# MartinMikkelsen/TensorTrainNumerics.jl

Hardware: AMD Instinct MI355X
Metric: TT cores/sec for QTT Laplacian apply+round, d=30 rank-64 (higher is better)
Workload: dtype f64

## Files before the change

### tensortrainnumerics.jl_amd/csrc/ttn_dense_kernels.h

```cpp
#pragma once
#include "ttn_wg_prims.h"
#include "ttn_wg_gemm.h"
#include "ttn_wg_lq.h"
#include "ttn_wg_jacobi.h"
#include "ttn_wg_chol.h"

struct CompressArgs {
    TTDev tt;
    long long max_bond;
    double truncerr;
    int sweeps;
    int k_single;
    int k_first, k_last;
    double* scratch;
    long long scratch_stride;
    int pmax, qmax;
    double* sv_out;
    int sv_steps;
    int* status;
    int* sweep_stats;
    int fast;
    int fused;
    TTODev op;
    TTDev x;
// ... 260 lines not shown
        const int i = e % r, j = e / r;
        const double si = S.sigs[i], sj = S.sigs[j];
        const double ref = (i == j) ? si * s0 : 0.0;
        worst = fmax(worst, fabs(D[i + (long long)ldd * j] - ref) / (s0 * sqrt(si * sj)));
    }
    return wg_max(worst, S.red);
}

__device__ void wg_materialize_core(const CompressArgs& P, int b, int k) {
    const TTDev& T = P.tt;
    const int n = T.dims[k];
    const long long* xr = P.x.rks + (long long)b * (P.x.d + 1);
    const int rl = uni32((int)xr[k]), rr = uni32((int)xr[k + 1]);
    const int Rl = uni32((int)P.op.rks[k]), Rr = uni32((int)P.op.rks[k + 1]);
    const double* xc = P.x.data + (long long)b * P.x.stride + P.x.off[k];
    const double* ac = P.op.data + P.op.off[k];
    double* yc = T.data + (long long)b * T.stride + T.off[k];
    const long long Dl = (long long)Rl * rl, tot = (long long)n * Dl * Rr * rr;
    for (long long e = threadIdx.x; e < tot; e += TTN_WG) {
        const int s = (int)(e % n);
        const long long t1 = e / n;
        const int ga = (int)(t1 % Dl), be = (int)(t1 / Dl);
        const int a1 = ga % Rl, nu1 = ga / Rl, a2 = be % Rr, nu2 = be / Rr;
        double v = 0.0;
        for (int j = 0; j < n; ++j)
            v = fma(ac[s + n * (j + n * (a1 + (long long)Rl * a2))], xc[j + n * (nu1 + (long long)rl * nu2)], v);
        yc[e] = v;
    }
    __syncthreads();
}

#define FM_BK 8
__device__ __noinline__ bool wg_fused_merge_mfma(double* ck, const double* xc, const double* ac, double* M, int p, int q, int n1, int Dl,
                                                 int rhl, int rhr, int Rl, int Rr, double* lds, double* amax_lds, double* red) {
    ck = unip(ck); xc = unip(xc); ac = unip(ac); M = unip(M); lds = unip(lds); amax_lds = unip(amax_lds); red = unip(red);
    p = uni32(p); q = uni32(q); n1 = uni32(n1); Dl = uni32(Dl); rhl = uni32(rhl); rhr = uni32(rhr); Rl = uni32(Rl); Rr = uni32(Rr);
    constexpr int n2 = 2;
    const int tid = threadIdx.x, lane = tid & 63, wave = tid >> 6;
    const int li = lane & 15, lk = lane >> 4;
    const int RT = p >> 4;
    const int WR = RT < 8 ? RT : 8;
    const int WC = TTN_NWAVES / WR;
    const int CP = 32 * WC;
    const int ncol = n2 * rhr, nin = Rl * n2, nout = n2 * Rr;
    constexpr int LDA = GEMM_LD;
    const int LDB = (CP <= 32) ? 49 : (CP <= 64) ? 81 : GEMM_LD;
    const int stage = Rl * FM_BK * LDA + FM_BK * LDB;
    if (Rl < 1 || Rl > 3 || Rr > 4 || (p & 15) || (rhl % FM_BK) || (ncol % CP) || (RT % WR) || WR * WC != TTN_NWAVES || CP > 128 ||
        Rl * FM_BK * 16 * WR > 6 * TTN_WG || FM_BK * CP > 2 * TTN_WG || 2 * stage + 64 > GEMM_LDS_DOUBLES)
        return false;
    lds_f64* opl = (lds_f64*)lds + 2 * stage;
    __syncthreads();
    for (int e = tid; e < nin * nout; e += TTN_WG) {
        const int i = e % nin, o = e / nin;
        opl[e] = ac[(o % n2) + n2 * ((i % n2) + n2 * ((i / n2) + (long long)Rl * (o / n2)))];
    }
    const long long ldk = (long long)n1 * Dl;
    const int wr = wave % WR, wc = wave / WR;
    const int nchunk = rhl / FM_BK;
    gmem_f64* Cg = (gmem_f64*)ck;
    gmem_f64* Xg = (gmem_f64*)xc;
    gmem_wf64* Mg = (gmem_wf64*)M;
    double cmax = 0.0;
    const int arows = 16 * WR;
    const int na_el = Rl * FM_BK * arows, nb_el = FM_BK * CP;
    constexpr int NUA = 6, NUB = 2;
    for (int rb = 0; rb < RT; rb += WR) {
        for (int c0 = 0; c0 < ncol; c0 += CP) {
            mfma_acc_t acc[3][2];
#pragma unroll
            for (int a1 = 0; a1 < 3; ++a1) { acc[a1][0] = (mfma_acc_t){0.0, 0.0, 0.0, 0.0}; acc[a1][1] = (mfma_acc_t){0.0, 0.0, 0.0, 0.0}; }
            int aoff[NUA], alds[NUA], boff[NUB], blds[NUB];
            bool aok[NUA], bok[NUB];
#pragma unroll
            for (int u = 0; u < NUA; ++u) {
                const int e = tid + TTN_WG * u;
                aok[u] = e < na_el;
                const int r = e % arows, rest = e / arows, kk = rest % FM_BK, a1 = rest / FM_BK;
                const int row = 16 * rb + r;
                aoff[u] = aok[u] ? (row % Dl) * n1 + row / Dl + (int)(ldk * (a1 + (long long)Rl * kk)) : 0;
                alds[u] = (a1 * FM_BK + kk) * LDA + r;
            }
#pragma unroll
            for (int u = 0; u < NUB; ++u) {
                const int e = tid + TTN_WG * u;
                bok[u] = e < nb_el;
                const int c = e % CP, kk = e / CP, col = c0 + c;
                boff[u] = bok[u] ? (col & 1) + n2 * (kk + rhl * (col >> 1)) : 0;
                blds[u] = kk * LDB + c;
            }
            const int astep = (int)(ldk * Rl * FM_BK), bstep = n2 * FM_BK;
            double av[NUA], bv[NUB];
#define FM_LOAD(CH)                                                                                                     \
            { _Pragma("unroll") for (int u = 0; u < NUA; ++u) av[u] = Cg[aoff[u] + (CH) * astep];                       \
              _Pragma("unroll") for (int u = 0; u < NUB; ++u) bv[u] = Xg[boff[u] + (CH) * bstep]; }
#define FM_STORE(STG)                                                                                                   \
            { lds_f64* As_ = (lds_f64*)lds + (STG) * stage; lds_f64* Bs_ = As_ + Rl * FM_BK * LDA;                      \
              _Pragma("unroll") for (int u = 0; u < NUA; ++u) if (aok[u]) As_[alds[u]] = av[u];                         \
              _Pragma("unroll") for (int u = 0; u < NUB; ++u) if (bok[u]) Bs_[blds[u]] = bv[u]; }
            __syncthreads();
            FM_LOAD(0)
            FM_STORE(0)
            if (nchunk > 1) FM_LOAD(1)
            __syncthreads();
            for (int ch = 0; ch < nchunk; ++ch) {
                const lds_f64* As = (lds_f64*)lds + (ch & 1) * stage;
                const lds_f64* Bs = As + Rl * FM_BK * LDA;
#pragma unroll
                for (int t = 0; t < FM_BK / 4; ++t) {
                    const int kr = 4 * t + lk;
                    const double b0 = Bs[kr * LDB + wc * 32 + li], b1 = Bs[kr * LDB + wc * 32 + 16 + li];
#pragma unroll
                    for (int a1 = 0; a1 < 3; ++a1) {
                        if (a1 < Rl) {
                            const double a = As[(a1 * FM_BK + kr) * LDA + wr * 16 + li];
                            acc[a1][0] = __builtin_amdgcn_mfma_f64_16x16x4f64(a, b0, acc[a1][0], 0, 0, 0);
                            acc[a1][1] = __builtin_amdgcn_mfma_f64_16x16x4f64(a, b1, acc[a1][1], 0, 0, 0);
                        }
                    }
                    if (t == 0 && ch + 1 < nchunk) FM_STORE((ch + 1) & 1)
                }
                if (ch + 2 < nchunk) FM_LOAD(ch + 2)
                __syncthreads();
            }
#undef FM_LOAD
#undef FM_STORE
            const int jl = li & 1;
#pragma unroll
            for (int ct = 0; ct < 2; ++ct) {
                const int nu = (c0 + wc * 32 + ct * 16 + li) >> 1;
#pragma unroll
                for (int reg = 0; reg < 4; ++reg) {
                    const int row = 16 * (rb + wr) + lk + 4 * reg;
                    gmem_wf64* mrow = Mg + ((long long)row * q + (long long)nout * nu);
                    for (int o = 0; o < nout; ++o) {
                        double v = 0.0;
#pragma unroll
                        for (int a1 = 0; a1 < 3; ++a1)
                            if (a1 < Rl) v = fma(acc[a1][ct][reg], opl[o * nin + jl + n2 * a1], v);
                        v += dpp_mov_f64<0xB1>(v);
                        if ((o & 1) == jl) mrow[o] = v;
                        cmax = fmax(cmax, fabs(v));
                    }
                }
            }
        }
    }
    cmax = wg_max(cmax, red);
    if (tid == 0) *amax_lds = cmax;
    __syncthreads();
    return true;
}

__device__ __noinline__ bool wg_fused_merge_direct(double* ck, const double* xc, const double* ac, double* M, int p, int q, int n1, int Dl,
                                                   int rhl, int rhr, int Rl, int Rr, double* lds, double* amax_lds, double* red) {
    ck = unip(ck); xc = unip(xc); ac = unip(ac); M = unip(M); lds = unip(lds); amax_lds = unip(amax_lds); red = unip(red);
    p = uni32(p); q = uni32(q); n1 = uni32(n1); Dl = uni32(Dl); rhl = uni32(rhl); rhr = uni32(rhr); Rl = uni32(Rl); Rr = uni32(Rr);
    constexpr int n2 = 2;
    const int tid = threadIdx.x, lane = tid & 63, wave = tid >> 6;
    const int li = lane & 15, lk = lane >> 4;
    const int RT = p >> 4;
    const int WR = RT < 8 ? RT : 8;
    const int WC = TTN_NWAVES / WR;
    const int CP = 32 * WC;
    const int ncol = n2 * rhr, nin = Rl * n2, nout = n2 * Rr;
    const int LDB = ncol + 1;
    if (Rl < 1 || Rl > 3 || Rr > 4 || (p & 15) || (rhl & 15) || (ncol % CP) || (RT % WR) || WR * WC != TTN_NWAVES ||
        (long long)rhl * LDB + 64 > GEMM_LDS_DOUBLES)
        return false;
    lds_f64* Bs = (lds_f64*)lds;
    lds_f64* opl = Bs + rhl * LDB;
    gmem_f64* Cg = (gmem_f64*)ck;
    gmem_f64* Xg = (gmem_f64*)xc;
    gmem_wf64* Mg = (gmem_wf64*)M;
    __syncthreads();
    for (int e = tid; e < nin * nout; e += TTN_WG) {
        const int i = e % nin, o = e / nin;
        opl[e] = ac[(o % n2) + n2 * ((i % n2) + n2 * ((i / n2) + (long long)Rl * (o / n2)))];
    }
    {
        const int nx = rhl * ncol, kspan = n2 * rhl;
        for (int e0 = tid; e0 < nx; e0 += 8 * TTN_WG) {
            double v[8];
#pragma unroll
            for (int u = 0; u < 8; ++u) { const int e = e0 + u * TTN_WG; v[u] = Xg[e < nx ? e : e0]; }
#pragma unroll
            for (int u = 0; u < 8; ++u) {
                const int e = e0 + u * TTN_WG;
                if (e < nx) { const int nu = e / kspan, w_ = e - nu * kspan, j = w_ & 1, kk = w_ >> 1; Bs[kk * LDB + j + n2 * nu] = v[u]; }
            }
        }
    }
    __syncthreads();
    const long long ldk = (long long)n1 * Dl;
    const int wr = wave % WR, wc = wave / WR;
    const int ksteps = rhl >> 2, ngrp = ksteps >> 2;
    const int kstride = (int)(ldk * Rl);
    double cmax = 0.0;
    const int jl = li & 1;
    for (int rb = 0; rb < RT; rb += WR) {
        const int arow = 16 * (rb + wr) + li;
        const int abase = (arow % Dl) * n1 + arow / Dl + lk * kstride;
        for (int c0 = 0; c0 < ncol; c0 += CP) {
            mfma_acc_t acc[3][2];
#pragma unroll
            for (int a1 = 0; a1 < 3; ++a1) { acc[a1][0] = (mfma_acc_t){0.0, 0.0, 0.0, 0.0}; acc[a1][1] = (mfma_acc_t){0.0, 0.0, 0.0, 0.0}; }
            double cur[4][3], nxt[4][3];
#define FMD_LOAD(DST, G)                                                                                                \
            _Pragma("unroll") for (int t = 0; t < 4; ++t)                                                                \
                _Pragma("unroll") for (int a1 = 0; a1 < 3; ++a1)                                                         \
                    DST[t][a1] = (a1 < Rl) ? Cg[abase + (4 * (4 * (G) + t)) * kstride + a1 * (int)ldk] : 0.0;
            FMD_LOAD(cur, 0)
            const lds_f64* bcol = Bs + lk * LDB + c0 + wc * 32 + li;
            for (int g = 0; g < ngrp; ++g) {
                if (g + 1 < ngrp) { FMD_LOAD(nxt, g + 1) }
#pragma unroll
                for (int t = 0; t < 4; ++t) {
                    const int kr = 4 * (4 * g + t);
                    const double b0 = bcol[kr * LDB], b1 = bcol[kr * LDB + 16];
#pragma unroll
                    for (int a1 = 0; a1 < 3; ++a1) {
                        if (a1 < Rl) {
                            acc[a1][0] = __builtin_amdgcn_mfma_f64_16x16x4f64(cur[t][a1], b0, acc[a1][0], 0, 0, 0);
                            acc[a1][1] = __builtin_amdgcn_mfma_f64_16x16x4f64(cur[t][a1], b1, acc[a1][1], 0, 0, 0);
                        }
                    }
                }
#pragma unroll
                for (int t = 0; t < 4; ++t)
#pragma unroll
                    for (int a1 = 0; a1 < 3; ++a1) cur[t][a1] = nxt[t][a1];
            }
#undef FMD_LOAD
            const int half = nout >> 1;
            const bool vec_ok = (half == 3) && ((((unsigned long long)Mg) & 15ull) == 0) && ((q & 1) == 0);
            if (vec_ok && Rl == 3) {
                double w[3][3][2];
#pragma unroll
                for (int oo = 0; oo < 3; ++oo)
#pragma unroll
                    for (int a1 = 0; a1 < 3; ++a1) {
                        const int o = 3 * jl + oo;
                        w[oo][a1][0] = opl[o * nin + jl + n2 * a1];
                        w[oo][a1][1] = opl[o * nin + (1 - jl) + n2 * a1];
                    }
                typedef double dbl2 __attribute__((ext_vector_type(2)));
                typedef __attribute__((address_space(1))) dbl2 gmem_wd2;
#pragma unroll
                for (int ct = 0; ct < 2; ++ct) {
                    const int nu = (c0 + wc * 32 + ct * 16 + li) >> 1;
#pragma unroll
                    for (int reg = 0; reg < 4; ++reg) {
                        const int row = 16 * (rb + wr) + lk + 4 * reg;
                        gmem_wf64* mrow = Mg + ((long long)row * q + (long long)nout * nu);
                        const double t0 = acc[0][ct][reg], t1 = acc[1][ct][reg], t2 = acc[2][ct][reg];
                        const double u0 = dpp_mov_f64<0xB1>(t0), u1 = dpp_mov_f64<0xB1>(t1), u2 = dpp_mov_f64<0xB1>(t2);
                        double v[3];
#pragma unroll
                        for (int oo = 0; oo < 3; ++oo) {
                            double x_ = t0 * w[oo][0][0];
                            x_ = fma(u0, w[oo][0][1], x_);
                            x_ = fma(t1, w[oo][1][0], x_); x_ = fma(u1, w[oo][1][1], x_);
                            x_ = fma(t2, w[oo][2][0], x_); x_ = fma(u2, w[oo][2][1], x_);
                            v[oo] = x_;
                            cmax = fmax(cmax, fabs(x_));
                        }
                        *(gmem_wd2*)(mrow + (jl ? 4 : 0)) = jl ? (dbl2){v[1], v[2]} : (dbl2){v[0], v[1]};
                        mrow[jl ? 3 : 2] = jl ? v[0] : v[2];
                    }
                }
            } else {
#pragma unroll
            for (int ct = 0; ct < 2; ++ct) {
                const int nu = (c0 + wc * 32 + ct * 16 + li) >> 1;
#pragma unroll
                for (int reg = 0; reg < 4; ++reg) {
                    const int row = 16 * (rb + wr) + lk + 4 * reg;
                    gmem_wf64* mrow = Mg + ((long long)row * q + (long long)nout * nu);
                    for (int o = 0; o < nout; ++o) {
                        double v = 0.0;
#pragma unroll
                        for (int a1 = 0; a1 < 3; ++a1)
                            if (a1 < Rl) v = fma(acc[a1][ct][reg], opl[o * nin + jl + n2 * a1], v);
                        v += dpp_mov_f64<0xB1>(v);
                        if ((o >= half) == (jl == 1)) mrow[o] = v;
                        cmax = fmax(cmax, fabs(v));
                    }
                }
            }
            }
        }
    }
    cmax = wg_max(cmax, red);
    if (tid == 0) *amax_lds = cmax;
    __syncthreads();
    return true;
}


#define FUSE_MAX_TERMS 16
__device__ bool wg_fused_merge(const CompressArgs& P, int b, int k, int p, int q, const View& Am, double* M, double* Tbuf,
                               long long tbuf_doubles, double* lds, double* amax_lds, double* red) {
    const TTDev& T = P.tt;
    const int n1 = T.dims[k], n2 = T.dims[k + 1];
    const long long* rks = T.rks + (long long)b * (T.d + 1);
    const int Dl = uni32((int)rks[k]);
    const long long* xr = P.x.rks + (long long)b * (P.x.d + 1);
    const int rhl = uni32((int)xr[k + 1]), rhr = uni32((int)xr[k + 2]);
    const int Rl = uni32((int)P.op.rks[k + 1]), Rr = uni32((int)P.op.rks[k + 2]);
    const int ncol = n2 * rhr;
    if (Rl * n2 > FUSE_MAX_TERMS || n2 * Rr > FUSE_MAX_TERMS || (long long)Rl * p * ncol > tbuf_doubles) return false;
    if ((long long)Rl * rhl != rks[k + 1] || (long long)n2 * Rr * rhr != q || p != n1 * Dl) return false;
    double* ck = T.data + (long long)b * T.stride + T.off[k];
    double* xc = P.x.data + (long long)b * P.x.stride + P.x.off[k + 1];
    const double* ac = P.op.data + P.op.off[k + 1];
    TTN_SETPRIO_GEMM();
    struct PrioRestore { __device__ ~PrioRestore() { TTN_SETPRIO_BASE(); } } prio_restore_;
    if (n2 == 2 && wg_fused_merge_direct(ck, xc, ac, M, p, q, n1, Dl, rhl, rhr, Rl, Rr, lds, amax_lds, red)) return true;
    if (n2 == 2 && wg_fused_merge_mfma(ck, xc, ac, M, p, q, n1, Dl, rhl, rhr, Rl, Rr, lds, amax_lds, red)) return true;
    const long long ldk = (long long)n1 * Dl;
    for (int a1 = 0; a1 < Rl; ++a1) {
        const View Av = mkview(ck + a1 * ldk, Am.r, plain((long long)Rl * ldk));
        const View Bv = mkview(xc, plain(n2), Idx{n2, 1, (long long)n2 * rhl});
        const View Cv = mkview(Tbuf + (long long)a1 * p * ncol, plain(ncol), plain(1));
        wg_gemm(p, ncol, rhl, Av, Bv, Cv, 1.0, 0.0, lds);
    }
    double mx = 0.0;
    const int nin = Rl * n2, nout = n2 * Rr;
    lds_f64* opl = (lds_f64*)lds;
    for (int e = threadIdx.x; e < nin * nout; e += TTN_WG) {
        const int i = e % nin, o = e / nin;
        opl[e] = ac[(o % n2) + n2 * ((i % n2) + n2 * ((i / n2) + (long long)Rl * (o / n2)))];
    }
    __syncthreads();
    const long long tstride = (long long)p * ncol;
    for (int e = threadIdx.x; e < p * rhr; e += TTN_WG) {
        const int nu = e % rhr, row = e / rhr;
        const double* tp = Tbuf + (long long)row * ncol + n2 * nu;
        double t[FUSE_MAX_TERMS];
#pragma unroll
        for (int i = 0; i < FUSE_MAX_TERMS; ++i) t[i] = (i < nin) ? tp[(i / n2) * tstride + (i % n2)] : 0.0;
        double* mrow = M + (long long)row * q + (long long)nout * nu;
        for (int o = 0; o < nout; ++o) {
            const lds_f64* w = opl + o * nin;
            double v = 0.0;
#pragma unroll
            for (int i = 0; i < FUSE_MAX_TERMS; ++i)
                if (i < nin) v = fma(t[i], w[i], v);
            mrow[o] = v;
            mx = fmax(mx, fabs(v));
        }
    }
    mx = wg_max(mx, red);
    if (threadIdx.x == 0) *amax_lds = mx;
    __syncthreads();
    return true;
}

#define SMALL_STEP_PMAX 8
#define SMALL_STEP_QMAX 256
struct SmallStepArgs {
    double truncerr;
    long long max_bond;
    int rank_rule, pmax;
    double* sv_row;
    int* status_b;
    double *red, *scal, *sigs;
    int *perm, *iflag;
};
__device__ __noinline__ int wg_bond_small(SmallStepArgs Q, double* ck, double* ck1, int n1, int n2, int Dl, int rm, int Dr, long long* rank_out, double* lds) {
    rm = uni32(rm); n1 = uni32(n1); n2 = uni32(n2); Dl = uni32(Dl); Dr = uni32(Dr);
    ck = unip(ck); ck1 = unip(ck1); rank_out = unip(rank_out); lds = unip(lds);
    const int mr = n1 * Dl, mc = n2 * Dr;
    const View Am = mkview(ck, Idx{Dl, (long long)n1, 1}, plain((long long)n1 * Dl));
    const View Bm = mkview(ck1, plain(n2), Idx{n2, 1, (long long)n2 * rm});
    const int wide = (mr <= mc) ? 1 : 0;
    const int p = wide ? mr : mc, q = wide ? mc : mr;
    const View Ap = wide ? Am : tview(Bm);
    const View Bp = wide ? Bm : tview(Am);
    Q.truncerr = unif64(Q.truncerr); Q.max_bond = uni64(Q.max_bond);
    Q.rank_rule = uni32(Q.rank_rule); Q.pmax = uni32(Q.pmax); Q.sv_row = unip(Q.sv_row); Q.status_b = unip(Q.status_b);
    Q.red = unip(Q.red); Q.scal = unip(Q.scal); Q.sigs = unip(Q.sigs); Q.perm = unip(Q.perm); Q.iflag = unip(Q.iflag);
    const int tid = threadIdx.x, lane = tid & 63, wave = tid >> 6;
    const int LDQ = q + 1;
    lds_f64* Ms = (lds_f64*)lds;
    lds_f64* Es = Ms + SMALL_STEP_PMAX * (SMALL_STEP_QMAX + 1);
    lds_f64* nr = Es + SMALL_STEP_PMAX * 17;
    lds_i32* flg = (lds_i32*)(nr + 16);
    gmem_f64* Ag = (gmem_f64*)Ap.p;
    gmem_f64* Bg = (gmem_f64*)Bp.p;
    __syncthreads();
    double mx = 0.0;
    for (int e = tid; e < p * q; e += TTN_WG) {
        const int i = e / q, j = e - i * q;
        const long long ao = ix(Ap.r, i), bo = ix(Bp.c, j);
        double acc = 0.0;
        for (int kk = 0; kk < rm; ++kk) acc = fma(Ag[ao + ix(Ap.c, kk)], Bg[bo + ix(Bp.r, kk)], acc);
        Ms[i * LDQ + j] = acc;
        mx = fmax(mx, fabs(acc));
    }
    for (int e = tid; e < p * 17; e += TTN_WG) Es[e] = ((e / 17) == (e % 17)) ? 1.0 : 0.0;
    mx = unif64(wg_max(mx, Q.red));
    const double s0 = (mx > 0.0) ? mx : 1.0, inv_s0 = 1.0 / s0;
    for (int e = tid; e < p * q; e += TTN_WG) { const int i = e / q, j = e - i * q; Ms[i * LDQ + j] *= inv_s0; }
    __syncthreads();
    double amax = 0.0;
    for (int i = wave; i < p; i += TTN_NWAVES) {
        double a = 0.0;
        for (int j = lane; j < q; j += 64) { const double v = Ms[i * LDQ + j]; a = fma(v, v, a); }
        a = wave_sum(a);
        if (lane == 0) nr[i] = a;
        amax = fmax(amax, a);
    }
    amax = unif64(wg_max(amax, Q.red));
    const double aneg = (double)q * DBL_EPSILON * DBL_EPSILON * amax;
    const double tol = sqrt((double)q) * DBL_EPSILON, tol2 = tol * tol;
    if (tid == 0) Q.scal[0] = aneg;
    const int pe = p + (p & 1), half = pe >> 1;
    int sweeps = 0, conv = (p < 2);
    for (; !conv && sweeps < JACOBI_MAX_SWEEPS; ++sweeps) {
        if (tid == 0) *flg = 0;
        __syncthreads();
        int rotated = 0;
        for (int round = 0; round < pe - 1; ++round) {
            for (int kk = wave; kk < half; kk += TTN_NWAVES) {
                int i, j;
                if (kk == 0) { i = round; j = pe - 1; }
                else { i = (round + kk) % (pe - 1); j = (round + pe - 1 - kk) % (pe - 1); }
                if (i > j) { const int t = i; i = j; j = t; }
                if (j >= p) continue;
                lds_f64* xi = Ms + i * LDQ;
                lds_f64* xj = Ms + j * LDQ;
                double u[4], v[4];
                double a = 0.0, b_ = 0.0, g = 0.0;
#pragma unroll
                for (int t4 = 0; t4 < 4; ++t4) {
                    const int c = lane + 64 * t4;
                    u[t4] = (c < q) ? xi[c] : 0.0; v[t4] = (c < q) ? xj[c] : 0.0;
                    a = fma(u[t4], u[t4], a); b_ = fma(v[t4], v[t4], b_); g = fma(u[t4], v[t4], g);
                }
                a = wave_sum(a); b_ = wave_sum(b_); g = wave_sum(g);
                if (a <= aneg || b_ <= aneg) continue;
                if (g * g <= tol2 * a * b_) continue;
                const double dd = b_ - a, hh = g + g;
                const double hyp = __builtin_amdgcn_sqrt(fma(dd, dd, hh * hh));
// ... 528 lines not shown
```

### tensortrainnumerics.jl_amd/csrc/ttn_wg_gemm.h

```cpp
#pragma once
#include "ttn_wg_prims.h"

#define GEMM_BK 16
#define GEMM_LD 145
#define GEMM_LDS_DOUBLES (TTN_LDS_IMG + 512)


struct GemmDesc {
    int m, n, k, pad;
    View A, B, C;
    double alpha, beta;
    unsigned long long* amax;
};
#if TTN_WG == 512
#define GEMM_TAB_ENTRIES 704
#define GEMM_KSLAB 512
#define GEMM_SMALL_KMAX 256
#else
#define GEMM_TAB_ENTRIES 1536
#define GEMM_KSLAB 768
#define GEMM_SMALL_KMAX 512
#endif
#define GEMM_DESC_DOUBLES (32 + GEMM_TAB_ENTRIES)
#define GEMM_LDS_TOTAL (GEMM_LDS_DOUBLES + GEMM_DESC_DOUBLES)

typedef __attribute__((address_space(3))) GemmDesc lds_gdesc;
__device__ inline Idx ldsIdx(const __attribute__((address_space(3))) Idx* d) { return Idx{uni32(d->q), uni64(d->lo), uni64(d->hi)}; }
__device__ inline View ldsView(const __attribute__((address_space(3))) View* v) { return View{(double*)uni64((long long)v->p), ldsIdx(&v->r), ldsIdx(&v->c)}; }

__device__ inline void gemm_publish_amax(const lds_gdesc* dsc, double cmax) {
    unsigned long long* am = (unsigned long long*)uni64((long long)dsc->amax);
    if (am) {
        cmax = wave_max(cmax);
        if ((threadIdx.x & 63) == 0) atomicMax(am, (unsigned long long)__double_as_longlong(cmax));
    }
}

template <int WR>
__device__ __noinline__ void wg_gemm_impl(const GemmDesc* dsc_, double* lds) {
    const lds_gdesc* dsc = (const lds_gdesc*)dsc_;
    constexpr int WCN = TTN_NWAVES / WR;
    constexpr int BM = 32 * WR, BN = 32 * WCN;
    constexpr int LDA = (BM <= 64) ? 81 : GEMM_LD, LDB = (BN <= 64) ? 81 : (BN <= 128) ? GEMM_LD : 273;
    constexpr int STAGE = GEMM_BK * (LDA + LDB);
    static_assert(2 * STAGE <= GEMM_LDS_DOUBLES, "two LDS stages must fit");
    const int m = uni32(dsc->m), n = uni32(dsc->n), k = uni32(dsc->k);
    const View A = ldsView(&dsc->A), B = ldsView(&dsc->B), C = ldsView(&dsc->C);
    const double alpha = unif64(dsc->alpha), beta = unif64(dsc->beta);
    const int tid = threadIdx.x, lane = tid & 63, wave = tid >> 6;
    const int wr = wave / WCN, wc = wave % WCN;
    const int li = lane & 15, lk = lane >> 4;
    gmem_f64* Ag = (gmem_f64*)A.p;
    gmem_f64* Bg = (gmem_f64*)B.p;
    lds_i32* tabA = (lds_i32*)(lds + GEMM_LDS_DOUBLES + 32);
    lds_i32* tabB = tabA + GEMM_KSLAB;
    const bool a_kfast = minstride(A.c) < minstride(A.r);
    const bool b_kfast = minstride(B.r) < minstride(B.c);
    constexpr int NUA = BM * GEMM_BK / TTN_WG, NUB = BN * GEMM_BK / TTN_WG;
    int ar[NUA], akk[NUA], bc[NUB], bkk[NUB];
#pragma unroll
    for (int u = 0; u < NUA; ++u) {
        const int e = tid + TTN_WG * u;
        if (a_kfast) { akk[u] = e & (GEMM_BK - 1); ar[u] = e / GEMM_BK; } else { ar[u] = e & (BM - 1); akk[u] = e / BM; }
    }
#pragma unroll
    for (int u = 0; u < NUB; ++u) {
        const int e = tid + TTN_WG * u;
        if (b_kfast) { bkk[u] = e & (GEMM_BK - 1); bc[u] = e / GEMM_BK; } else { bc[u] = e & (BN - 1); bkk[u] = e / BN; }
    }
    double cmax = 0.0;
    const int nch = (k + GEMM_BK - 1) / GEMM_BK;
    int slab0 = -1;
    for (int m0 = 0; m0 < m; m0 += BM) {
        for (int n0 = 0; n0 < n; n0 += BN) {
            int aoff[NUA], boff[NUB];
            bool aok[NUA], bok[NUB];
#pragma unroll
            for (int u = 0; u < NUA; ++u) { aok[u] = (m0 + ar[u]) < m; aoff[u] = aok[u] ? (int)ix(A.r, m0 + ar[u]) : 0; }
#pragma unroll
            for (int u = 0; u < NUB; ++u) { bok[u] = (n0 + bc[u]) < n; boff[u] = bok[u] ? (int)ix(B.c, n0 + bc[u]) : 0; }
            const bool live = (m0 + wr * 32 < m) && (n0 + wc * 32 < n);
            mfma_acc_t acc[2][2];
#pragma unroll
            for (int i = 0; i < 2; ++i)
#pragma unroll
                for (int j = 0; j < 2; ++j) acc[i][j] = (mfma_acc_t){0.0, 0.0, 0.0, 0.0};
            double av[NUA], bv[NUB];
#define GEMM_FILL_TAB(K0)                                                                                       \
            {                                                                                                   \
                __syncthreads();                                                                                \
                slab0 = (K0);                                                                                   \
                for (int j = tid; j < GEMM_KSLAB; j += TTN_WG) {                                                \
                    const int kk = slab0 + j;                                                                   \
                    tabA[j] = (kk < k) ? (int)ix(A.c, kk) : 0;                                                     \
                    tabB[j] = (kk < k) ? (int)ix(B.r, kk) : 0;                                                     \
                }                                                                                               \
                __syncthreads();                                                                                \
            }
#define GEMM_LOAD(K0)          \
            {                                                                                                   \
                int oa_[NUA], ob_[NUB];                                                                         \
                bool va_[NUA], vb_[NUB];                                                                        \
                _Pragma("unroll") for (int u = 0; u < NUA; ++u) {                                               \
                    const int ga = (K0) + akk[u];                                                               \
                    va_[u] = aok[u] && ga < k;                                                                  \
                    oa_[u] = va_[u] ? aoff[u] + tabA[ga - slab0] : 0;                                           \
                }                                                                                               \
                _Pragma("unroll") for (int u = 0; u < NUB; ++u) {                                               \
                    const int gb = (K0) + bkk[u];                                                               \
                    vb_[u] = bok[u] && gb < k;                                                                  \
                    ob_[u] = vb_[u] ? boff[u] + tabB[gb - slab0] : 0;                                           \
                }                                                                                               \
                _Pragma("unroll") for (int u = 0; u < NUA; ++u) av[u] = Ag[oa_[u]];                             \
                _Pragma("unroll") for (int u = 0; u < NUB; ++u) bv[u] = Bg[ob_[u]];                             \
                _Pragma("unroll") for (int u = 0; u < NUA; ++u) av[u] = va_[u] ? av[u] : 0.0;                   \
                _Pragma("unroll") for (int u = 0; u < NUB; ++u) bv[u] = vb_[u] ? bv[u] : 0.0;                   \
            }
#define GEMM_STORE(STG)                                                                                         \
            {                                                                                                   \
                lds_f64* As_ = (lds_f64*)lds + (STG) * STAGE;                                                    \
                lds_f64* Bs_ = As_ + GEMM_BK * LDA;                                                             \
                _Pragma("unroll") for (int u = 0; u < NUA; ++u) As_[akk[u] * LDA + ar[u]] = av[u];              \
                _Pragma("unroll") for (int u = 0; u < NUB; ++u) Bs_[bkk[u] * LDB + bc[u]] = bv[u];              \
            }
            if (slab0 != 0) GEMM_FILL_TAB(0)
            else __syncthreads();
            {
                GEMM_LOAD(0)
                double av0[NUA], bv0[NUB];
                _Pragma("unroll") for (int u = 0; u < NUA; ++u) av0[u] = av[u];
                _Pragma("unroll") for (int u = 0; u < NUB; ++u) bv0[u] = bv[u];
                if (nch > 1) GEMM_LOAD(GEMM_BK)
                lds_f64* As0 = (lds_f64*)lds;
                lds_f64* Bs0 = As0 + GEMM_BK * LDA;
                _Pragma("unroll") for (int u = 0; u < NUA; ++u) As0[akk[u] * LDA + ar[u]] = av0[u];
                _Pragma("unroll") for (int u = 0; u < NUB; ++u) Bs0[bkk[u] * LDB + bc[u]] = bv0[u];
            }
            __syncthreads();
            for (int c = 0; c < nch; ++c) {
                lds_f64* As = (lds_f64*)lds + (c & 1) * STAGE;
                lds_f64* Bs = As + GEMM_BK * LDA;
#define GEMM_MFMA_STEP(T)                                                                                       \
                if (live) {                                                                                     \
                    const int kra = (4 * (T) + lk) * LDA, krb = (4 * (T) + lk) * LDB;                                                 \
                    const double a0 = As[kra + wr * 32 + li], a1 = As[kra + wr * 32 + 16 + li];                 \
                    const double b0 = Bs[krb + wc * 32 + li], b1 = Bs[krb + wc * 32 + 16 + li];                 \
                    acc[0][0] = __builtin_amdgcn_mfma_f64_16x16x4f64(a0, b0, acc[0][0], 0, 0, 0);               \
                    acc[0][1] = __builtin_amdgcn_mfma_f64_16x16x4f64(a0, b1, acc[0][1], 0, 0, 0);               \
                    acc[1][0] = __builtin_amdgcn_mfma_f64_16x16x4f64(a1, b0, acc[1][0], 0, 0, 0);               \
                    acc[1][1] = __builtin_amdgcn_mfma_f64_16x16x4f64(a1, b1, acc[1][1], 0, 0, 0);               \
                }
                GEMM_MFMA_STEP(0)
                if (c + 1 < nch) GEMM_STORE((c + 1) & 1)
                GEMM_MFMA_STEP(1)
                if (c + 2 < nch) {
                    const int k2 = (c + 2) * GEMM_BK;
                    if (k2 >= slab0 + GEMM_KSLAB) GEMM_FILL_TAB(k2)
                    GEMM_LOAD(k2)
                }
                GEMM_MFMA_STEP(2)
                GEMM_MFMA_STEP(3)
#undef GEMM_MFMA_STEP
                __syncthreads();
            }
#undef GEMM_FILL_TAB
#undef GEMM_LOAD
#undef GEMM_STORE
            lds_i32* rowC = tabB + GEMM_KSLAB;
            lds_i32* colC = rowC + BM;
            for (int i = tid; i < BM + BN; i += TTN_WG) {
                if (i < BM) rowC[i] = (m0 + i < m) ? (int)ix(C.r, m0 + i) : 0;
                else colC[i - BM] = (n0 + i - BM < n) ? (int)ix(C.c, n0 + i - BM) : 0;
            }
            __syncthreads();
            if (live) {
#pragma unroll
                for (int ti = 0; ti < 2; ++ti)
#pragma unroll
                    for (int reg = 0; reg < 4; ++reg) {
                        const int li_ = wr * 32 + ti * 16 + lk + 4 * reg;
                        if (m0 + li_ >= m) continue;
                        const int ro = rowC[li_];
#pragma unroll
                        for (int tj = 0; tj < 2; ++tj) {
                            const int lj_ = wc * 32 + tj * 16 + li;
                            if (n0 + lj_ >= n) continue;
                            gmem_wf64* cp = (gmem_wf64*)C.p + ((long long)ro + colC[lj_]);
                            double v = alpha * acc[ti][tj][reg];
                            if (beta != 0.0) v += beta * (*cp);
                            *cp = v;
                            cmax = fmax(cmax, fabs(v));
                        }
                    }
            }
        }
    }
    gemm_publish_amax(dsc, cmax);
    __syncthreads();
}

__device__ inline int small_ld(int x) { const int t = (x + 15) & ~15; return (((t & 31) == 16) ? t : t + 16) + 1; }
__device__ inline int tight_ld(int x) { return ((x + 15) & ~15) + 1; }

__device__ __noinline__ void wg_gemm_small_impl(const GemmDesc* dsc_, double* lds) {
    const lds_gdesc* dsc = (const lds_gdesc*)dsc_;
    const int m = uni32(dsc->m), n = uni32(dsc->n), k = uni32(dsc->k);
    const View A = ldsView(&dsc->A), B = ldsView(&dsc->B), C = ldsView(&dsc->C);
    const double alpha = unif64(dsc->alpha), beta = unif64(dsc->beta);
    const int tid = threadIdx.x, lane = tid & 63, wave = tid >> 6;
    const int li = lane & 15, lk = lane >> 4;
    const int lda = uni32(dsc->pad) ? small_ld(m) : tight_ld(m), ldb = uni32(dsc->pad) ? small_ld(n) : tight_ld(n);
    lds_f64* As = (lds_f64*)lds;
    lds_f64* Bs = As + k * lda;
    const bool a_kfast = minstride(A.c) < minstride(A.r);
    const bool b_kfast = minstride(B.r) < minstride(B.c);
    const int mp = (m + 15) & ~15, np = (n + 15) & ~15;
    gmem_f64* Ag = (gmem_f64*)A.p;
    gmem_f64* Bg = (gmem_f64*)B.p;
    lds_i32* rowA = (lds_i32*)(lds + GEMM_LDS_DOUBLES + 32);
    lds_i32* colB = rowA + 128;
    lds_i32* rowC = colB + 128;
    lds_i32* colC = rowC + 128;
    lds_i32* kA = colC + 128;
    lds_i32* kB = kA + GEMM_SMALL_KMAX;
    for (int i = tid; i < 128; i += TTN_WG) {
        rowA[i] = (i < m) ? (int)ix(A.r, i) : 0;
        rowC[i] = (i < m) ? (int)ix(C.r, i) : 0;
        colB[i] = (i < n) ? (int)ix(B.c, i) : 0;
        colC[i] = (i < n) ? (int)ix(C.c, i) : 0;
    }
    for (int i = tid; i < k; i += TTN_WG) { kA[i] = (int)ix(A.c, i); kB[i] = (int)ix(B.r, i); }
    __syncthreads();
    const int fx = tid & 15, sy = tid >> 4;
#define GS_U 8
#define GEMM_SMALL_STAGE(DST, LDD, SRC, SLOWTAB, FASTTAB, NSLOW, NSLOW_VALID, NFAST, NFAST_VALID, SLOW_IS_K)                      \
    for (int s_ = sy; s_ < (NSLOW); s_ += TTN_WG / 16) {                                                                        \
        const int so_ = (s_ < (NSLOW_VALID)) ? SLOWTAB[s_] : 0;                                                                 \
        for (int f0_ = fx; f0_ < (NFAST); f0_ += 16 * GS_U) {                                                                   \
            double v_[GS_U];                                                                                                    \
            _Pragma("unroll") for (int u_ = 0; u_ < GS_U; ++u_) {                                                               \
                const int f_ = f0_ + 16 * u_;                                                                                   \
                const bool ok_ = (s_ < (NSLOW_VALID)) && (f_ < (NFAST_VALID));                                                  \
                v_[u_] = SRC[ok_ ? so_ + FASTTAB[f_] : 0];                                                                      \
            }                                                                                                                   \
            _Pragma("unroll") for (int u_ = 0; u_ < GS_U; ++u_) {                                                               \
                const int f_ = f0_ + 16 * u_;                                                                                   \
                const bool ok_ = (s_ < (NSLOW_VALID)) && (f_ < (NFAST_VALID));                                                  \
                if (f_ < (NFAST)) DST[(SLOW_IS_K) ? s_ * (LDD) + f_ : f_ * (LDD) + s_] = ok_ ? v_[u_] : 0.0;                    \
            }                                                                                                                   \
        }                                                                                                                       \
    }
    if (a_kfast) { GEMM_SMALL_STAGE(As, lda, Ag, rowA, kA, mp, m, k, k, 0) }
    else { GEMM_SMALL_STAGE(As, lda, Ag, kA, rowA, k, k, mp, m, 1) }
    if (b_kfast) { GEMM_SMALL_STAGE(Bs, ldb, Bg, colB, kB, np, n, k, k, 0) }
    else { GEMM_SMALL_STAGE(Bs, ldb, Bg, kB, colB, k, k, np, n, 1) }
#undef GEMM_SMALL_STAGE
#undef GS_U
    __syncthreads();
    const int tm = mp >> 4, tn = np >> 4, ntile = tm * tn;
    const int k4 = k >> 2, krem = k & 3;
    double cmax = 0.0;
    for (int tile = wave; tile < ntile; tile += (TTN_WG >> 6)) {
        const int r0 = (tile % tm) << 4, c0 = (tile / tm) << 4;
        mfma_acc_t acc = (mfma_acc_t){0.0, 0.0, 0.0, 0.0};
        const lds_f64* ap = As + lk * lda + r0 + li;
        const lds_f64* bp = Bs + lk * ldb + c0 + li;
        int t = 0;
        for (; t + 4 <= k4; t += 4) {
            double a_[4], b_[4];
#pragma unroll
            for (int q = 0; q < 4; ++q) { a_[q] = ap[(4 * (t + q)) * lda]; b_[q] = bp[(4 * (t + q)) * ldb]; }
#pragma unroll
            for (int q = 0; q < 4; ++q) acc = __builtin_amdgcn_mfma_f64_16x16x4f64(a_[q], b_[q], acc, 0, 0, 0);
        }
        for (; t < k4; ++t) acc = __builtin_amdgcn_mfma_f64_16x16x4f64(ap[(4 * t) * lda], bp[(4 * t) * ldb], acc, 0, 0, 0);
        if (krem) {
            const double a = (lk < krem) ? ap[(4 * k4) * lda] : 0.0;
            const double b = (lk < krem) ? bp[(4 * k4) * ldb] : 0.0;
            acc = __builtin_amdgcn_mfma_f64_16x16x4f64(a, b, acc, 0, 0, 0);
        }
#pragma unroll
        for (int reg = 0; reg < 4; ++reg) {
            const int gi = r0 + lk + 4 * reg, gj = c0 + li;
            if (gi < m && gj < n) {
                gmem_wf64* cp = (gmem_wf64*)C.p + ((long long)rowC[gi] + colC[gj]);
                double v = alpha * acc[reg];
                if (beta != 0.0) v += beta * (*cp);
                *cp = v;
                cmax = fmax(cmax, fabs(v));
            }
        }
    }
    gemm_publish_amax(dsc, cmax);
    __syncthreads();
}

__device__ inline void wg_gemm(int m, int n, int k, View A, View B, View C, double alpha, double beta, double* lds,
                               double* amax_lds = nullptr ) {
    GemmDesc* dsc = reinterpret_cast<GemmDesc*>(lds + GEMM_LDS_DOUBLES);
    __syncthreads();
    if (threadIdx.x == 0) {
        dsc->m = m; dsc->n = n; dsc->k = k; dsc->pad = 0;
        dsc->A = A; dsc->B = B; dsc->C = C;
        dsc->alpha = alpha; dsc->beta = beta;
        dsc->amax = (unsigned long long*)amax_lds;
        if (amax_lds) *amax_lds = 0.0;
    }
    __syncthreads();
    TTN_SETPRIO_GEMM();
    const bool shape_ok = (m <= 128) && (n <= 128) && (((m + 15) >> 4) * ((n + 15) >> 4) <= 32);
    const int wpad = small_ld(m) + small_ld(n), wtight = tight_ld(m) + tight_ld(n);
    if (shape_ok && (long long)k * wpad <= GEMM_LDS_DOUBLES) {
        if (threadIdx.x == 0) dsc->pad = 1;
        __syncthreads();
        wg_gemm_small_impl(dsc, lds);
    } else if (shape_ok && (long long)k * wtight <= GEMM_LDS_DOUBLES) {
        wg_gemm_small_impl(dsc, lds);
    } else if (shape_ok && A.c.q == 0 && B.r.q == 0 && k <= 8 * (GEMM_LDS_DOUBLES / wtight)) {
        const int kcmax = (GEMM_LDS_DOUBLES / wtight) & ~3;
        const int nck = (k + kcmax - 1) / kcmax;
        const int kc = (((k + nck - 1) / nck) + 3) & ~3;
        for (int k0 = 0; k0 < k; k0 += kc) {
            if (k0 > 0) __syncthreads();
            if (threadIdx.x == 0) {
                dsc->k = (k - k0 < kc) ? k - k0 : kc;
                dsc->A.p = A.p + ix(A.c, k0);
                dsc->B.p = B.p + ix(B.r, k0);
                dsc->beta = (k0 == 0) ? beta : 1.0;
                dsc->amax = (k0 + kc >= k) ? (unsigned long long*)amax_lds : nullptr;
            }
            __syncthreads();
            wg_gemm_small_impl(dsc, lds);
        }
    } else if (m <= 64 && n > 128) {
        wg_gemm_impl<2>(dsc, lds);
    } else {
        wg_gemm_impl<4>(dsc, lds);
    }
    TTN_SETPRIO_BASE();
}

#define SYRK_QMAX (2 * GEMM_TAB_ENTRIES - 128)
template <int KC16, int JMAX, int MAXT>
__device__ __noinline__ void wg_syrk_impl(const GemmDesc* dsc_, double* lds) {
    const lds_gdesc* dsc = (const lds_gdesc*)dsc_;
    constexpr int KC = 16 * KC16, RG = TTN_WG / 16;
    const int p = uni32(dsc->m), q = uni32(dsc->k);
    const View A = ldsView(&dsc->A), C = ldsView(&dsc->C);
    const double alpha = unif64(dsc->alpha);
// ... 184 lines not shown
```

Baseline: 595,300.

## Template fused-merge tile loop on Rl and cut register pressure in GEMM staging

Result: faster. 614,200, median of 6 (+3.2%).

```diff
diff --git a/tensortrainnumerics.jl_amd/csrc/ttn_dense_kernels.h b/tensortrainnumerics.jl_amd/csrc/ttn_dense_kernels.h
--- a/tensortrainnumerics.jl_amd/csrc/ttn_dense_kernels.h
+++ b/tensortrainnumerics.jl_amd/csrc/ttn_dense_kernels.h
@@ -436,13 +436,144 @@
     return true;
 }
 
+typedef unsigned int fmd_u32x2 __attribute__((ext_vector_type(2)));
+__device__ __forceinline__ double fmd_ld(__amdgpu_buffer_rsrc_t rs, unsigned voff, unsigned soff) {
+    return __builtin_bit_cast(double, (fmd_u32x2)__builtin_amdgcn_raw_buffer_load_b64(rs, (int)voff, (int)soff, 0));
+}
+template <int RL>
+__device__ __forceinline__ double fmd_tiles(gmem_f64* Cg, gmem_wf64* Mg, const lds_f64* Bs, const lds_f64* opl, int p, int q, int n1,
+                                            int Dl, int rhl, int rhr, int Rr, int LDB) {
+    constexpr int n2 = 2, nin = RL * n2;
+    const int tid = threadIdx.x, lane = tid & 63, wave = tid >> 6;
+    const int li = lane & 15, lk = lane >> 4;
+    const int RT = p >> 4;
+    const int WR = RT < 8 ? RT : 8;
+    const int WC = TTN_NWAVES / WR;
+    const int CP = 32 * WC;
+    const int ncol = n2 * rhr, nout = n2 * Rr;
+    const int ldk = n1 * Dl;
+    const int wr = uni32(wave % WR), wc = uni32(wave / WR);
+    const int ngrp = rhl >> 4;
+    const int kstride = ldk * RL;
+    const unsigned a_step = 8u * (unsigned)ldk, t_step = 8u * (unsigned)(4 * kstride - (RL - 1) * ldk);
+    double cmax = 0.0;
+    const __amdgpu_buffer_rsrc_t crs = __builtin_amdgcn_make_buffer_rsrc((void*)Cg, 0, 8 * kstride * rhl, 0x00020000);
+    for (int rb = 0; rb < RT; rb += WR) {
+        const int arow = 16 * (rb + wr) + li;
+        const unsigned aoff = 8u * (unsigned)((arow % Dl) * n1 + arow / Dl + lk * kstride);
+        for (int c0 = 0; c0 < ncol; c0 += CP) {
+            mfma_acc_t acc[RL][2];
+#pragma unroll
+            for (int a1 = 0; a1 < RL; ++a1) { acc[a1][0] = (mfma_acc_t){0.0, 0.0, 0.0, 0.0}; acc[a1][1] = (mfma_acc_t){0.0, 0.0, 0.0, 0.0}; }
+            double fa[4][RL], fb[4][RL];
+            const lds_f64* bp = Bs + lk * LDB + c0 + wc * 32 + li;
+#define FMD_LOAD(DST, G)      \
+            {                                                                                                           \
+                unsigned so_ = 8u * (unsigned)(16 * (G) * kstride);                                                     \
+                _Pragma("unroll") for (int t = 0; t < 4; ++t)                                                            \
+                    _Pragma("unroll") for (int a1 = 0; a1 < RL; ++a1) {                                                  \
+                        DST[t][a1] = fmd_ld(crs, aoff, so_);                                                            \
+                        so_ += (a1 + 1 < RL) ? a_step : t_step;                                                         \
+                        asm volatile("" : "+s"(so_));                                                                   \
+                    }                                                                                                   \
+            }
+#define FMD_MFMA(SRC, G)                                                                                                \
+            _Pragma("unroll") for (int t = 0; t < 4; ++t) {                                                              \
+                const double b0 = bp[0], b1 = bp[16];                                                                   \
+                bp += 4 * LDB;                                                                                          \
+                asm volatile("" : "+v"(bp));          \
+                _Pragma("unroll") for (int a1 = 0; a1 < RL; ++a1) {                                                      \
+                    acc[a1][0] = __builtin_amdgcn_mfma_f64_16x16x4f64(SRC[t][a1], b0, acc[a1][0], 0, 0, 0);             \
+                    acc[a1][1] = __builtin_amdgcn_mfma_f64_16x16x4f64(SRC[t][a1], b1, acc[a1][1], 0, 0, 0);             \
+                }                                                                                                       \
+            }
+            FMD_LOAD(fa, 0)
+            int g = 0;
+            for (; g + 2 < ngrp; g += 2) {
+                FMD_LOAD(fb, g + 1)
+                FMD_MFMA(fa, g)
+                FMD_LOAD(fa, g + 2)
+                FMD_MFMA(fb, g + 1)
+            }
+            {
+                const bool two = g + 1 < ngrp;
+                FMD_LOAD(fb, two ? g + 1 : g)
+                FMD_MFMA(fa, g)
+                if (two) { FMD_MFMA(fb, g + 1) }
+            }
+#undef FMD_LOAD
+#undef FMD_MFMA
+            int te = tid;
+            asm volatile("" : "+v"(te));
+            const int lie = te & 15, lke = (te >> 4) & 3, jl = lie & 1;
+            const int half = nout >> 1;
+            const bool vec_ok = (half == 3) && ((((unsigned long long)Mg) & 15ull) == 0) && ((q & 1) == 0);
+            if (RL == 3 && vec_ok) {
+                constexpr int R3 = RL == 3 ? 3 : 1;
+                double w[3][R3][2];
+#pragma unroll
+                for (int oo = 0; oo < 3; ++oo)
+#pragma unroll
+                    for (int a1 = 0; a1 < R3; ++a1) {
+                        const int o = 3 * jl + oo;
+                        w[oo][a1][0] = opl[o * nin + jl + n2 * a1];
+                        w[oo][a1][1] = opl[o * nin + (1 - jl) + n2 * a1];
+                    }
+                typedef double dbl2 __attribute__((ext_vector_type(2)));
+                typedef __attribute__((address_space(1))) dbl2 gmem_wd2;
+#pragma unroll
+                for (int ct = 0; ct < 2; ++ct) {
+                    const int nu = (c0 + wc * 32 + ct * 16 + lie) >> 1;
+#pragma unroll
+                    for (int reg = 0; reg < 4; ++reg) {
+                        const int row = 16 * (rb + wr) + lke + 4 * reg;
+                        gmem_wf64* mrow = Mg + ((long long)row * q + (long long)nout * nu);
+                        const double t0 = acc[0][ct][reg], t1 = acc[R3 > 1 ? 1 : 0][ct][reg], t2 = acc[R3 > 2 ? 2 : 0][ct][reg];
+                        const double u0 = dpp_mov_f64<0xB1>(t0), u1 = dpp_mov_f64<0xB1>(t1), u2 = dpp_mov_f64<0xB1>(t2);
+                        double v[3];
+#pragma unroll
+                        for (int oo = 0; oo < 3; ++oo) {
+                            double x_ = t0 * w[oo][0][0];
+                            x_ = fma(u0, w[oo][0][1], x_);
+                            x_ = fma(t1, w[oo][R3 > 1 ? 1 : 0][0], x_); x_ = fma(u1, w[oo][R3 > 1 ? 1 : 0][1], x_);
+                            x_ = fma(t2, w[oo][R3 > 2 ? 2 : 0][0], x_); x_ = fma(u2, w[oo][R3 > 2 ? 2 : 0][1], x_);
+                            v[oo] = x_;
+                            cmax = fmax(cmax, fabs(x_));
+                        }
+                        *(gmem_wd2*)(mrow + (jl ? 4 : 0)) = jl ? (dbl2){v[1], v[2]} : (dbl2){v[0], v[1]};
+                        mrow[jl ? 3 : 2] = jl ? v[0] : v[2];
+                    }
+                }
+            } else {
+#pragma unroll
+                for (int ct = 0; ct < 2; ++ct) {
+                    const int nu = (c0 + wc * 32 + ct * 16 + lie) >> 1;
+#pragma unroll
+                    for (int reg = 0; reg < 4; ++reg) {
+                        const int row = 16 * (rb + wr) + lke + 4 * reg;
+                        gmem_wf64* mrow = Mg + ((long long)row * q + (long long)nout * nu);
+                        for (int o = 0; o < nout; ++o) {
+                            double v = 0.0;
+#pragma unroll
+                            for (int a1 = 0; a1 < RL; ++a1) v = fma(acc[a1][ct][reg], opl[o * nin + jl + n2 * a1], v);
+                            v += dpp_mov_f64<0xB1>(v);
+                            if ((o >= half) == (jl == 1)) mrow[o] = v;
+                            cmax = fmax(cmax, fabs(v));
+                        }
+                    }
+                }
+            }
+        }
+    }
+    return cmax;
+}
+
 __device__ __noinline__ bool wg_fused_merge_direct(double* ck, const double* xc, const double* ac, double* M, int p, int q, int n1, int Dl,
                                                    int rhl, int rhr, int Rl, int Rr, double* lds, double* amax_lds, double* red) {
     ck = unip(ck); xc = unip(xc); ac = unip(ac); M = unip(M); lds = unip(lds); amax_lds = unip(amax_lds); red = unip(red);
     p = uni32(p); q = uni32(q); n1 = uni32(n1); Dl = uni32(Dl); rhl = uni32(rhl); rhr = uni32(rhr); Rl = uni32(Rl); Rr = uni32(Rr);
     constexpr int n2 = 2;
-    const int tid = threadIdx.x, lane = tid & 63, wave = tid >> 6;
-    const int li = lane & 15, lk = lane >> 4;
+    const int tid = threadIdx.x;
     const int RT = p >> 4;
     const int WR = RT < 8 ? RT : 8;
     const int WC = TTN_NWAVES / WR;
@@ -476,105 +607,10 @@
         }
     }
     __syncthreads();
-    const long long ldk = (long long)n1 * Dl;
-    const int wr = wave % WR, wc = wave / WR;
-    const int ksteps = rhl >> 2, ngrp = ksteps >> 2;
-    const int kstride = (int)(ldk * Rl);
-    double cmax = 0.0;
-    const int jl = li & 1;
-    for (int rb = 0; rb < RT; rb += WR) {
-        const int arow = 16 * (rb + wr) + li;
-        const int abase = (arow % Dl) * n1 + arow / Dl + lk * kstride;
-        for (int c0 = 0; c0 < ncol; c0 += CP) {
-            mfma_acc_t acc[3][2];
-#pragma unroll
-            for (int a1 = 0; a1 < 3; ++a1) { acc[a1][0] = (mfma_acc_t){0.0, 0.0, 0.0, 0.0}; acc[a1][1] = (mfma_acc_t){0.0, 0.0, 0.0, 0.0}; }
-            double cur[4][3], nxt[4][3];
-#define FMD_LOAD(DST, G)                                                                                                \
-            _Pragma("unroll") for (int t = 0; t < 4; ++t)                                                                \
-                _Pragma("unroll") for (int a1 = 0; a1 < 3; ++a1)                                                         \
-                    DST[t][a1] = (a1 < Rl) ? Cg[abase + (4 * (4 * (G) + t)) * kstride + a1 * (int)ldk] : 0.0;
-            FMD_LOAD(cur, 0)
-            const lds_f64* bcol = Bs + lk * LDB + c0 + wc * 32 + li;
-            for (int g = 0; g < ngrp; ++g) {
-                if (g + 1 < ngrp) { FMD_LOAD(nxt, g + 1) }
-#pragma unroll
-                for (int t = 0; t < 4; ++t) {
-                    const int kr = 4 * (4 * g + t);
-                    const double b0 = bcol[kr * LDB], b1 = bcol[kr * LDB + 16];
-#pragma unroll
-                    for (int a1 = 0; a1 < 3; ++a1) {
-                        if (a1 < Rl) {
-                            acc[a1][0] = __builtin_amdgcn_mfma_f64_16x16x4f64(cur[t][a1], b0, acc[a1][0], 0, 0, 0);
-                            acc[a1][1] = __builtin_amdgcn_mfma_f64_16x16x4f64(cur[t][a1], b1, acc[a1][1], 0, 0, 0);
-                        }
-                    }
-                }
-#pragma unroll
-                for (int t = 0; t < 4; ++t)
-#pragma unroll
-                    for (int a1 = 0; a1 < 3; ++a1) cur[t][a1] = nxt[t][a1];
-            }
-#undef FMD_LOAD
-            const int half = nout >> 1;
-            const bool vec_ok = (half == 3) && ((((unsigned long long)Mg) & 15ull) == 0) && ((q & 1) == 0);
-            if (vec_ok && Rl == 3) {
-                double w[3][3][2];
-#pragma unroll
-                for (int oo = 0; oo < 3; ++oo)
-#pragma unroll
-                    for (int a1 = 0; a1 < 3; ++a1) {
-                        const int o = 3 * jl + oo;
-                        w[oo][a1][0] = opl[o * nin + jl + n2 * a1];
-                        w[oo][a1][1] = opl[o * nin + (1 - jl) + n2 * a1];
-                    }
-                typedef double dbl2 __attribute__((ext_vector_type(2)));
-                typedef __attribute__((address_space(1))) dbl2 gmem_wd2;
-#pragma unroll
-                for (int ct = 0; ct < 2; ++ct) {
-                    const int nu = (c0 + wc * 32 + ct * 16 + li) >> 1;
-#pragma unroll
-                    for (int reg = 0; reg < 4; ++reg) {
-                        const int row = 16 * (rb + wr) + lk + 4 * reg;
-                        gmem_wf64* mrow = Mg + ((long long)row * q + (long long)nout * nu);
-                        const double t0 = acc[0][ct][reg], t1 = acc[1][ct][reg], t2 = acc[2][ct][reg];
-                        const double u0 = dpp_mov_f64<0xB1>(t0), u1 = dpp_mov_f64<0xB1>(t1), u2 = dpp_mov_f64<0xB1>(t2);
-                        double v[3];
-#pragma unroll
-                        for (int oo = 0; oo < 3; ++oo) {
-                            double x_ = t0 * w[oo][0][0];
-                            x_ = fma(u0, w[oo][0][1], x_);
-                            x_ = fma(t1, w[oo][1][0], x_); x_ = fma(u1, w[oo][1][1], x_);
-                            x_ = fma(t2, w[oo][2][0], x_); x_ = fma(u2, w[oo][2][1], x_);
-                            v[oo] = x_;
-                            cmax = fmax(cmax, fabs(x_));
-                        }
-                        *(gmem_wd2*)(mrow + (jl ? 4 : 0)) = jl ? (dbl2){v[1], v[2]} : (dbl2){v[0], v[1]};
-                        mrow[jl ? 3 : 2] = jl ? v[0] : v[2];
-                    }
-                }
-            } else {
-#pragma unroll
-            for (int ct = 0; ct < 2; ++ct) {
-                const int nu = (c0 + wc * 32 + ct * 16 + li) >> 1;
-#pragma unroll
-                for (int reg = 0; reg < 4; ++reg) {
-                    const int row = 16 * (rb + wr) + lk + 4 * reg;
-                    gmem_wf64* mrow = Mg + ((long long)row * q + (long long)nout * nu);
-                    for (int o = 0; o < nout; ++o) {
-                        double v = 0.0;
-#pragma unroll
-                        for (int a1 = 0; a1 < 3; ++a1)
-                            if (a1 < Rl) v = fma(acc[a1][ct][reg], opl[o * nin + jl + n2 * a1], v);
-                        v += dpp_mov_f64<0xB1>(v);
-                        if ((o >= half) == (jl == 1)) mrow[o] = v;
-                        cmax = fmax(cmax, fabs(v));
-                    }
-                }
-            }
-            }
-        }
-    }
+    double cmax;
+    if (Rl == 3) cmax = fmd_tiles<3>(Cg, Mg, Bs, opl, p, q, n1, Dl, rhl, rhr, Rr, LDB);
+    else if (Rl == 2) cmax = fmd_tiles<2>(Cg, Mg, Bs, opl, p, q, n1, Dl, rhl, rhr, Rr, LDB);
+    else cmax = fmd_tiles<1>(Cg, Mg, Bs, opl, p, q, n1, Dl, rhl, rhr, Rr, LDB);
     cmax = wg_max(cmax, red);
     if (tid == 0) *amax_lds = cmax;
     __syncthreads();
diff --git a/tensortrainnumerics.jl_amd/csrc/ttn_wg_gemm.h b/tensortrainnumerics.jl_amd/csrc/ttn_wg_gemm.h
--- a/tensortrainnumerics.jl_amd/csrc/ttn_wg_gemm.h
+++ b/tensortrainnumerics.jl_amd/csrc/ttn_wg_gemm.h
@@ -57,28 +57,35 @@
     const bool a_kfast = minstride(A.c) < minstride(A.r);
     const bool b_kfast = minstride(B.r) < minstride(B.c);
     constexpr int NUA = BM * GEMM_BK / TTN_WG, NUB = BN * GEMM_BK / TTN_WG;
-    int ar[NUA], akk[NUA], bc[NUB], bkk[NUB];
-#pragma unroll
-    for (int u = 0; u < NUA; ++u) {
-        const int e = tid + TTN_WG * u;
-        if (a_kfast) { akk[u] = e & (GEMM_BK - 1); ar[u] = e / GEMM_BK; } else { ar[u] = e & (BM - 1); akk[u] = e / BM; }
-    }
-#pragma unroll
-    for (int u = 0; u < NUB; ++u) {
-        const int e = tid + TTN_WG * u;
-        if (b_kfast) { bkk[u] = e & (GEMM_BK - 1); bc[u] = e / GEMM_BK; } else { bc[u] = e & (BN - 1); bkk[u] = e / BN; }
-    }
+    static_assert(TTN_WG % BM == 0 && TTN_WG % BN == 0 && TTN_WG % GEMM_BK == 0, "the staging steps are uniform");
+    const int ars = a_kfast ? TTN_WG / GEMM_BK : 0, aks = a_kfast ? 0 : TTN_WG / BM;
+    const int bcs = b_kfast ? TTN_WG / GEMM_BK : 0, bks = b_kfast ? 0 : TTN_WG / BN;
+    constexpr int LBK = 4, LBM = BM == 64 ? 6 : 7, LBN = BN == 64 ? 6 : BN == 128 ? 7 : 8;
+    static_assert((1 << LBK) == GEMM_BK && (1 << LBM) == BM && (1 << LBN) == BN, "powers of two");
+    const int arsh = a_kfast ? LBK : 0, armk = a_kfast ? -1 : BM - 1, aksh = a_kfast ? 0 : LBM, akmk = a_kfast ? GEMM_BK - 1 : -1;
+    const int bcsh = b_kfast ? LBK : 0, bcmk = b_kfast ? -1 : BN - 1, bksh = b_kfast ? 0 : LBN, bkmk = b_kfast ? GEMM_BK - 1 : -1;
+#define GEMM_IDX                                                                                                \
+    int t_ = tid;                                                                                               \
+    asm volatile("" : "+v"(t_));                                                                                \
+    const int ar0 = (t_ >> arsh) & armk, akk0 = (t_ >> aksh) & akmk;                                            \
+    const int bc0 = (t_ >> bcsh) & bcmk, bkk0 = (t_ >> bksh) & bkmk;
+#define AR(u) (ar0 + ars * (u))
+#define AKK(u) (akk0 + aks * (u))
+#define BC(u) (bc0 + bcs * (u))
+#define BKK(u) (bkk0 + bks * (u))
     double cmax = 0.0;
     const int nch = (k + GEMM_BK - 1) / GEMM_BK;
     int slab0 = -1;
     for (int m0 = 0; m0 < m; m0 += BM) {
         for (int n0 = 0; n0 < n; n0 += BN) {
             int aoff[NUA], boff[NUB];
-            bool aok[NUA], bok[NUB];
-#pragma unroll
-            for (int u = 0; u < NUA; ++u) { aok[u] = (m0 + ar[u]) < m; aoff[u] = aok[u] ? (int)ix(A.r, m0 + ar[u]) : 0; }
-#pragma unroll
-            for (int u = 0; u < NUB; ++u) { bok[u] = (n0 + bc[u]) < n; boff[u] = bok[u] ? (int)ix(B.c, n0 + bc[u]) : 0; }
+            {
+                GEMM_IDX
+#pragma unroll
+                for (int u = 0; u < NUA; ++u) aoff[u] = (m0 + AR(u)) < m ? (int)ix(A.r, m0 + AR(u)) : 0;
+#pragma unroll
+                for (int u = 0; u < NUB; ++u) boff[u] = (n0 + BC(u)) < n ? (int)ix(B.c, n0 + BC(u)) : 0;
+            }
             const bool live = (m0 + wr * 32 < m) && (n0 + wc * 32 < n);
             mfma_acc_t acc[2][2];
 #pragma unroll
@@ -99,16 +106,17 @@
             }
 #define GEMM_LOAD(K0)          \
             {                                                                                                   \
+                GEMM_IDX                                                                                        \
                 int oa_[NUA], ob_[NUB];                                                                         \
                 bool va_[NUA], vb_[NUB];                                                                        \
                 _Pragma("unroll") for (int u = 0; u < NUA; ++u) {                                               \
-                    const int ga = (K0) + akk[u];                                                               \
-                    va_[u] = aok[u] && ga < k;                                                                  \
+                    const int ga = (K0) + AKK(u);                                                               \
+                    va_[u] = (m0 + AR(u)) < m && ga < k;                                                        \
                     oa_[u] = va_[u] ? aoff[u] + tabA[ga - slab0] : 0;                                           \
                 }                                                                                               \
                 _Pragma("unroll") for (int u = 0; u < NUB; ++u) {                                               \
-                    const int gb = (K0) + bkk[u];                                                               \
-                    vb_[u] = bok[u] && gb < k;                                                                  \
+                    const int gb = (K0) + BKK(u);                                                               \
+                    vb_[u] = (n0 + BC(u)) < n && gb < k;                                                        \
                     ob_[u] = vb_[u] ? boff[u] + tabB[gb - slab0] : 0;                                           \
                 }                                                                                               \
                 _Pragma("unroll") for (int u = 0; u < NUA; ++u) av[u] = Ag[oa_[u]];                             \
@@ -118,10 +126,11 @@
             }
 #define GEMM_STORE(STG)                                                                                         \
             {                                                                                                   \
+                GEMM_IDX                                                                                        \
                 lds_f64* As_ = (lds_f64*)lds + (STG) * STAGE;                                                    \
                 lds_f64* Bs_ = As_ + GEMM_BK * LDA;                                                             \
-                _Pragma("unroll") for (int u = 0; u < NUA; ++u) As_[akk[u] * LDA + ar[u]] = av[u];              \
-                _Pragma("unroll") for (int u = 0; u < NUB; ++u) Bs_[bkk[u] * LDB + bc[u]] = bv[u];              \
+                _Pragma("unroll") for (int u = 0; u < NUA; ++u) As_[AKK(u) * LDA + AR(u)] = av[u];              \
+                _Pragma("unroll") for (int u = 0; u < NUB; ++u) Bs_[BKK(u) * LDB + BC(u)] = bv[u];              \
             }
             if (slab0 != 0) GEMM_FILL_TAB(0)
             else __syncthreads();
@@ -131,10 +140,11 @@
                 _Pragma("unroll") for (int u = 0; u < NUA; ++u) av0[u] = av[u];
                 _Pragma("unroll") for (int u = 0; u < NUB; ++u) bv0[u] = bv[u];
                 if (nch > 1) GEMM_LOAD(GEMM_BK)
+                GEMM_IDX
                 lds_f64* As0 = (lds_f64*)lds;
                 lds_f64* Bs0 = As0 + GEMM_BK * LDA;
-                _Pragma("unroll") for (int u = 0; u < NUA; ++u) As0[akk[u] * LDA + ar[u]] = av0[u];
-                _Pragma("unroll") for (int u = 0; u < NUB; ++u) Bs0[bkk[u] * LDB + bc[u]] = bv0[u];
+                _Pragma("unroll") for (int u = 0; u < NUA; ++u) As0[AKK(u) * LDA + AR(u)] = av0[u];
+                _Pragma("unroll") for (int u = 0; u < NUB; ++u) Bs0[BKK(u) * LDB + BC(u)] = bv0[u];
             }
             __syncthreads();
             for (int c = 0; c < nch; ++c) {
@@ -195,6 +205,11 @@
             }
         }
     }
+#undef GEMM_IDX
+#undef AR
+#undef AKK
+#undef BC
+#undef BKK
     gemm_publish_amax(dsc, cmax);
     __syncthreads();
 }
```
